# CloudEngineHub/MARL-LLM

Measured on AMD Instinct MI355X. Metric: agent-steps/sec, higher is better.
Workload: dtype f64 (state, every index / flag / reward decision) + f32 (obs, prior, action I/O, pre-filters); 1 GPU; assembly env, 64 agents x 4096 envs per GPU (64 x 4096 total), assembled state, prior-policy actions; agents=64, envs_per_gpu=4096, envs_total=4096, obs_dtype=f32, state_dtype=f64, seed=226, parallelism=env-sharded x1, no collective on the step path

## Files before the change

### marl_llm_amd/csrc/swarm_env.hip

```cpp

#include <hip/hip_runtime.h>

#include <cmath>
#include <cstdint>
#include <cstring>
#include <string>
#include <type_traits>
#include <utility>

#include "swarm_env.h"
#include "env_types.h"

using namespace swarm_internal;

namespace {

typedef unsigned long long u64;

typedef float f2v __attribute__((ext_vector_type(2)));

template <typename T> struct Pair;
template <> struct Pair<float>  { typedef float2 type; };
template <> struct Pair<double> { typedef double2 type; };
typedef __attribute__((ext_vector_type(2))) __bf16 bf2v;
// ... 60 lines not shown
        "v_addc_co_u32_e64 %2, %8, %2, %2, %8\n\t"
        "v_addc_co_u32_e64 %3, %9, %3, %3, %9\n\t"
        "v_addc_co_u32_e64 %4, %10, %4, %4, %10\n\t"
        "v_addc_co_u32_e64 %5, %11, %5, %5, %11"
        : "+v"(nb), "+v"(hi), "+v"(ht), "+v"(cd), "+v"(c1), "+v"(c2), "=&s"(m0), "=&s"(m1), "=&s"(m2), "=&s"(m3), "=&s"(m4), "=&s"(m5)
        : "v"(d2u), "v"(d2), "s"(c_nb), "s"(c_hi), "s"(c_ht), "s"(c_cd), "s"(c_c1), "s"(c_c2));
}

template <typename F, int... I>
__device__ __forceinline__ void static_for_impl(F &&f, std::integer_sequence<int, I...>)
{
    (f(std::integral_constant<int, I>{}), ...);
}
template <int N, typename F>
__device__ __forceinline__ void static_for(F &&f)
{
    static_for_impl(static_cast<F &&>(f), std::make_integer_sequence<int, N>{});
}

__device__ __forceinline__ double clamp_ref(double v, double lo, double hi)
{
    double m = (hi < v) ? hi : v;
    return (lo < m) ? m : lo;
}

#define REPS(k) ((P.dbg_phase == (k)) ? P.dbg_extra + 1 : 1)
#define FENCE() asm volatile("" ::: "memory")
#define EXIT_AT(k) do { if (P.dbg_phase == 15 && P.dbg_extra == (k)) return; } while (0)

#ifdef SWARM_STAMPS
#define STAMP(k) do { __builtin_amdgcn_sched_barrier(0); if (P.stamps != nullptr && (threadIdx.x & 63) == 0) P.stamps[((size_t)blockIdx.x * (blockDim.x >> 6) + (threadIdx.x >> 6)) * 24 + (k)] = clock64(); __builtin_amdgcn_sched_barrier(0); } while (0)
#else
#define STAMP(k) do { } while (0)
#endif

template <int NPAD, bool HALF = false> struct Geo {
    static_assert(!HALF || NPAD < 64, "the half-occupied geometry is for N < 64");
    static constexpr int NPAD_ = NPAD; static constexpr bool HALF_ = HALF;
    static constexpr bool CT_MAP = NPAD >= 64 || HALF;
    static constexpr int AG = NPAD < 64 ? 64 : NPAD;
    static constexpr int EPB = NPAD < 64 ? (64 / NPAD) / (HALF ? 2 : 1) : 1;
    static constexpr int ACTW = NPAD < 64 ? EPB * NPAD : 64;
    static constexpr int LPA = HALF ? 8 : 4;
    static constexpr int AGW = 64 / LPA;
    static constexpr int NW = AG / 64;
    static constexpr int WPE = 4;
    static constexpr int T = AG * WPE;
#ifndef SWARM_WPS
#define SWARM_WPS 7
#endif
#ifndef SWARM_WPS_SMALL
#define SWARM_WPS_SMALL 6
#endif
#ifndef SWARM_WPS_128
#define SWARM_WPS_128 6
#endif
    static constexpr int WPS_LAT = NPAD == 64 ? SWARM_WPS : (NPAD < 64 ? SWARM_WPS_SMALL : (NPAD == 128 ? SWARM_WPS_128 : 1));
    static constexpr int WPS_GEN = NPAD == 64 ? 6 : (NPAD < 64 ? 5 : 1);
};

template <int NPAD, bool HALF> struct LatMap {
    typedef Geo<NPAD, HALF> G_;
    static constexpr int AG = G_::AG, EPB = G_::EPB, NW = G_::NW, WPE = G_::WPE, T = G_::T;
    static constexpr int NRC = 16;
    static constexpr int al(int bytes) { return (bytes + 15) & ~15; }
    static constexpr int mx(int a, int b) { return a > b ? a : b; }
    static constexpr int sp_bytes = 4 * AG * 8;
    static constexpr int hdr_bytes = AG * 16;
    static constexpr int rew_scratch_bytes = NW * 1536;
    static constexpr int srow_bytes = mx((NRC - 1) * AG * 4, rew_scratch_bytes);
    static constexpr int pcr_bytes = AG * NRC;
    static constexpr int partc_bytes = WPE * AG * 2;
    static constexpr int partd_bytes = (WPE - 1) * AG * 8;
    static constexpr int lat_bytes = EPB * 64 * (8 + 2);
    static constexpr int cov_bytes = EPB * 64 * 8;
    static constexpr int flag_bytes = AG;
    static constexpr int snei_bytes = AG * kNeiStride * 2;
    static constexpr int sncf_bytes = AG * 4;
    static constexpr int snear_bytes = NW > 1 ? NW * AG * 8 : 0;
    static constexpr int orow_bytes = NRC * AG * 4;
    static constexpr int pm_bytes = (NW == 1 ? WPE * 4 : 5) * NW * AG * 8;
    static constexpr int sp = 0;
    static constexpr int hdr = sp + al(sp_bytes);
    static constexpr int srow = hdr + al(hdr_bytes);
    static constexpr int pcr = srow + al(srow_bytes);
    static constexpr int partc = pcr + al(pcr_bytes);
    static constexpr int partd = partc + al(partc_bytes);
    static constexpr int lat = partd + al(partd_bytes);
    static constexpr int cov = lat + al(lat_bytes);
    static constexpr int flag = cov + al(cov_bytes);
    static constexpr int snei = flag + al(flag_bytes);
// ... 91 lines not shown
    unsigned *cov = reinterpret_cast<unsigned *>(smem + LO(cov));
    int *sflag = reinterpret_cast<int *>(smem + LO(flag));
    unsigned char *pc = smem + P.off_pc;
    constexpr int NRC = LM::NRC;
    float4 *hdr = reinterpret_cast<float4 *>(smem + LO(hdr));
    unsigned *srow = reinterpret_cast<unsigned *>(smem + LO(srow));
    unsigned char *pcr = smem + LO(pcr);
    u64 *covrow = reinterpret_cast<u64 *>(smem + LO(cov));
    unsigned char *perm = smem + LO(perm);
    unsigned *orow = reinterpret_cast<unsigned *>(smem + P.off_orow);

    if constexpr (FILT) {
        bool any_zero = false;
        for (int k = 0; k < EPB; ++k) {
            const int ek = blockIdx.x * EPB + k;
            any_zero = any_zero || P.lat[ek < P.n_env ? ek : P.n_env - 1].nrows == 0;
        }
        if (any_zero == LAT) return;
    }
    const int tid = threadIdx.x, lane = tid & 63;
    STAMP(0);
    const int at = tid % AG;
    const int sx = __builtin_amdgcn_readfirstlane((tid / AG + (int)blockIdx.x) % WPE);
    const int aw = at >> 6;
    auto flag_get = [&]() -> bool { return LAT ? ((reinterpret_cast<const unsigned *>(sflag)[at >> 2] >> ((at & 3) * 8)) & 1u) != 0 : (sflag[at] & 1) != 0; };
    const bool thr_on = NPAD >= 64 || at < ACTW;
    const int el = (NPAD < 64 && thr_on) ? at / NPAD : 0;
    const int i = NPAD < 64 ? at % NPAD : at;
    const int e = blockIdx.x * EPB + el;
    const int n_a = P.n_a;
    const bool act = thr_on && (e < P.n_env) && (i < n_a);
    const int es = e < P.n_env ? e : P.n_env - 1;
    const int ng = P.n_g[es];
    int ngb = ng;
    if (EPB > 1) {
        for (int k = 0; k < EPB; ++k) {
            const int ek = blockIdx.x * EPB + k;
            const int v = P.n_g[ek < P.n_env ? ek : P.n_env - 1];
            ngb = v > ngb ? v : ngb;
        }
    }
    const int W = (ngb + 31) >> 5;
    constexpr int SB = WPE > 1 ? 1 : 0;
    int w0 = W;
    if (WPE > 1) { w0 = (W - 2 * (WPE - 1)) / WPE; w0 = w0 < 0 ? 0 : w0; }
    auto mine = [&](int w) -> bool {
        if (WPE == 1) return true;
        if (w < w0) return sx == SB;
        const int o = (w - w0) % (WPE - 1);
        return sx == (o < SB ? o : o + 1);
    };
    const double2 *gce = P.cells_xy + (size_t)es * P.ng_max;
    auto cell64 = [&](int c) -> double2 { double2 g = gce[c < ng ? c : 0]; if (!(c < ng)) { g.x = kSentinel; g.y = kSentinel; } return g; };
    const float *cq_e = cxq + (size_t)el * P.cxq_stride;

    const size_t sbase = (size_t)es * 2 * n_a;
    double px = __builtin_nan(""), py = __builtin_nan(""), vx = 0.0, vy = 0.0;
    double ax = 0.0, ay = 0.0;
    double sf0x = 0.0, sf0y = 0.0;
    OT2 pri_now; pri_now.x = to_out<OT>(0.0); pri_now.y = to_out<OT>(0.0);
    const bool copy_prior = DO_STEP && P.with_prior && a_prior != nullptr;
    if (sx == 0 && act) {
        if (DO_STEP) { const double2 sfl = P.sf_next[(size_t)e * n_a + i]; sf0x = sfl.x; sf0y = sfl.y; }
        px = P.p[sbase + i]; py = P.p[sbase + n_a + i];
        vx = P.dp[sbase + i]; vy = P.dp[sbase + n_a + i];
        if (DO_STEP) {
// ... 367 lines not shown
            const bool c0 = fmaf(e0, e0, dy2) < ri2, c1 = fmaf(e1, e1, dy2) < ri2;
            MT acc = range(ao0, ao1);
            MT bnd = (MT)((c0 ? (MT)0 : (MT)1 << (ao0 & (MB - 1))) | (c1 ? (MT)0 : (MT)1 << (ao1 & (MB - 1)))) & acc & rowm;
            acc &= ~bnd;
            while (__any(bnd != 0)) {
                if (bnd != 0) {
                    const int a = ffs0(bnd);
                    bnd &= bnd - 1;
                    const int c = rst + popc(rowm & (MT)(((MT)1 << a) - 1));
                    const double2 g = cell64(c);
                    const double ex = g.x - px, ey = g.y - py;
                    if (ex * ex + ey * ey < cut) acc |= (MT)1 << a;
                }
            }
            return rowm & acc;
        };
        for (int rep = 0, reps = REPS(3); rep < reps; ++rep) {
            FENCE();
            for (int t = wr; t < P.lat_nrs; t += WS)
                srow[t * AG + at] = (unsigned)(row_sel(b0s + t, L.R, P.c_sen) >> ca0);
            const int b0c = (int)ceilf(bpf - (L.Rc + 2.0f * lat_m));
            for (int t = wr; t < P.lat_nrc; t += WS) {
                const MT selc = row_sel(b0c + t, L.Rc, P.c_occ);
                const int bq = b0c + t < 0 ? 0 : (b0c + t > 63 ? 63 : b0c + t);
                if (selc != 0) {
                    if constexpr (MB == 32) atomicOr(reinterpret_cast<unsigned *>(&covrow[el * 64 + bq]), (unsigned)selc);
                    else atomicOr(reinterpret_cast<unsigned long long *>(&covrow[el * 64 + bq]), (unsigned long long)selc);
                }
            }
            best32 = INFINITY; second32 = INFINITY; bc = 0;
            const int ar0 = (int)floorf(apf) + 1;
            const int a_r = ar0 < 0 ? 0 : (ar0 > MB - 1 ? MB - 1 : ar0);
            const MT lowm = (MT)(((MT)1 << a_r) - 1);
            const int nr_hi = EPB == 1 ? nrows : 64;
            auto row_cands = [&](int b, float &d2d, float &d2u, int &c_dn) {
                const MT rowm = (EPB == 1 || b < nrows) ? rowmask(b) : (MT)0;
                const float dy = (float)b - bpf, dy2 = dy * dy;
                const MT up = rowm >> a_r, dn = rowm & lowm;
                const int a_up = a_r + ffs0(up);
                const int a_dn = MB - 1 - (MB == 32 ? __clz((int)dn) : __clzll((long long)dn));
                const float dxu = (float)a_up - apf, dxd = (float)a_dn - apf;
                d2u = (act && up != 0) ? fmaf(dxu, dxu, dy2) : INFINITY;
                d2d = (act && dn != 0) ? fmaf(dxd, dxd, dy2) : INFINITY;
                c_dn = rs[b] + popc(dn) - 1;
            };
            for (int b = wr; b < nr_hi; b += WS) {
                float d2d, d2u; int c_dn;
                row_cands(b, d2d, d2u, c_dn);
                second32 = __builtin_amdgcn_fmed3f(best32, second32, d2d);
                bool lt = d2d < best32;
                best32 = lt ? d2d : best32; bc = lt ? c_dn : bc;
                second32 = __builtin_amdgcn_fmed3f(best32, second32, d2u);
                lt = d2u < best32;
                best32 = lt ? d2u : best32; bc = lt ? c_dn + 1 : bc;
            }
            const float lat_dlt = 1.2e-7f * fmaxf(fabsf(apf), fabsf(bpf)) + 2e-6f;
            const float tol = 6.0f * sqrtf(second32) * lat_dlt + 1e-9f;
            const bool unc_min = act && (wave_exact || (second32 < INFINITY && (second32 - best32) <= tol));
            if (__any(unc_min)) {
                if (unc_min) {
                    const float thr = wave_exact ? INFINITY : best32 + tol;
                    double bestd = INFINITY; int bcd = bc;
                    for (int b = wr; b < nr_hi; b += WS) {
                        float d2d, d2u; int c_dn;
                        row_cands(b, d2d, d2u, c_dn);
                        const bool td = d2d <= thr, tu = d2u <= thr && d2u < INFINITY;
                        if ((td && d2d < INFINITY) || tu) {
                            const double2 g0 = cell64((td && d2d < INFINITY) ? c_dn : 0), g1 = cell64(tu ? c_dn + 1 : 0);
                            const double e0x = g0.x - px, e0y = g0.y - py, e1x = g1.x - px, e1y = g1.y - py;
                            const double q0 = e0x * e0x + e0y * e0y, q1 = e1x * e1x + e1y * e1y;
                            if (td && d2d < INFINITY && q0 < bestd) { bestd = q0; bcd = c_dn; }
                            if (tu && q1 < bestd) { bestd = q1; bcd = c_dn + 1; }
                        }
                    }
                    bc = bcd;
                }
            }
        }
        };
        if (sx != SB || WPE == 1) { if (P.lat_n32) walk(0u); else walk((u64)0); }
    } else
    for (int rep = 0, reps = REPS(3); rep < reps; ++rep) {
    FENCE();
    best32 = INFINITY; second32 = INFINITY; bc = 0;
    for (int w = 0; w < W; ++w) {
        if (!mine(w)) continue;
        unsigned word = 0, rword = 0;
        int mlo = 0, mhi = 0;
        int bl = 0; const float best_in = best32;
        unsigned orw = 0;
        const unsigned nlo = (unsigned)nearby1, nhi = (unsigned)(nearby1 >> 32);
        u64 unc = 0;
        const float4 *cq = reinterpret_cast<const float4 *>(cq_e + w * 64);
        static_for<16>([&](auto prc) {
            constexpr int pr = decltype(prc)::value;
            const float4 q = cq[pr];
            const f2v gx = {q.x, q.y}, gy = {q.z, q.w};
            const f2v rx = gx - pxx, ry = gy - pyy;
            const f2v d2v = __builtin_elementwise_fma(rx, rx, ry * ry);
            static_for<2>([&](auto hc) {
                constexpr int hh = decltype(hc)::value;
                constexpr int b = 2 * pr + hh;
                const float d2 = hh ? d2v.y : d2v.x;
                second32 = __builtin_amdgcn_fmed3f(best32, second32, d2);
                const bool lt = d2 < best32;
                best32 = lt ? d2 : best32;
                bl = lt ? b : bl;
                const u64 m_slo = __ballot(d2 < P.csen_lo), m_shi = __ballot(d2 < P.csen_hi);
                const u64 m_olo = __ballot(d2 < P.cocc_lo), m_ohi = __ballot(d2 < P.cocc_hi);
                rword = shl1_or_mask(rword, m_slo);
                if constexpr (NW == 1) {
                    const unsigned t = ((unsigned)m_olo & nlo) | ((unsigned)(m_olo >> 32) & nhi);
                    orw = shl1_or_mask(orw, __ballot(t != 0));
// ... 46 lines not shown
                }
            }
            if (unc_min) bc = bcd;
        }
    }
    part_c[sx * AG + at] = (pc_t)bc;
    double *part_d = reinterpret_cast<double *>(smem + LO(partd));
    if constexpr (LAT) {
        if (sx != SB || WPE == 1) {
            const double2 g = cell64(bc);
            const double ex = g.x - px, ey = g.y - py;
            part_d[(WPE > 1 && sx > SB ? sx - 1 : sx) * AG + at] = ex * ex + ey * ey;
        }
    }
    STAMP(16);
    EXIT_AT(4);
    __syncthreads();
    STAMP(17);
    double best = INFINITY; bc = 0;
    for (int rep = 0, reps = REPS(12); rep < reps; ++rep) {
    FENCE();
    best = INFINITY; bc = 0;
#pragma unroll
    for (int s = 0; s < WPE; ++s) {
        if (LAT && WPE > 1 && s == SB) continue;
        const int c = part_c[s * AG + at];
        double d;
        if constexpr (LAT) d = part_d[(WPE > 1 && s > SB ? s - 1 : s) * AG + at];
        else { const double2 g = cell64(c); const double ex = g.x - px, ey = g.y - py; d = ex * ex + ey * ey; }
        if (d < best || (d == best && c < bc)) { best = d; bc = c; }
    }
    }
    const bool in_shape = act && best < P.c_in[es];
    if (sx == 0) {
        sncf[at] = bc | (in_shape ? (1 << 30) : 0);
        if (P.export_small && act) {
            P.near_cell[(size_t)e * n_a + i] = bc;
            P.in_flag[(size_t)e * n_a + i] = in_shape ? 1 : 0;
        }
    }
    STAMP(4);
    EXIT_AT(5);

    const int PPR = P.obs_dim >> 1;
    const int HP = 2 * (P.with_self + P.topo) + 2;
    const int envs_here = (P.n_env - blockIdx.x * EPB) < EPB ? (P.n_env - blockIdx.x * EPB) : EPB;
    const int rows = envs_here * n_a;
    OT2 *out = reinterpret_cast<OT2 *>(obs) + (size_t)blockIdx.x * EPB * n_a * PPR;

    auto prior_policy = [&]() {
    if (sx == SB && P.with_prior) {
        double qx = 0.0, qy = 0.0;
        double lx = 0.0, ly = 0.0;
        {
            const int ncf = sncf[at];
            double tx = px - px, ty = py - py;
            if (!(ncf >> 30)) { const double2 g = cell64(ncf & 0xFFFF); tx = g.x - px; ty = g.y - py; }
            const double dt_ = sqrt(tx * tx + ty * ty);
            if (dt_ > 0) { qx += P.pk_att * tx / dt_; qy += P.pk_att * ty / dt_; }
            lx = qx; ly = qy;
            double avx = 0.0, avy = 0.0; int cnt = 0;
#pragma unroll
            for (int k = 0; k < kTopoMax; ++k) {
                const int j = snei[at * kNeiStride + k];
                const bool used = j >= 0;
                const int tj = el * NPAD + (used ? j : 0);
                const double x = px - sp[tj], y = py - sp[AG + tj];
                const double d2n = x * x + y * y;
                if (used && d2n > 0 && d2n < P.c_avoid) {
                    const double d = sqrt(d2n);
                    const double ux = x / d, uy = y / d;
                    const double factor = P.pk_rep * (P.r_avoid / d - 1.0);
// ... 947 lines not shown
```

### marl_llm_amd/csrc/env_api.hip

```cpp

#include <hip/hip_runtime.h>

#include <algorithm>
#include <cmath>
#include <cstddef>
#include <cstdint>
#include <cstring>
#include <new>
#include <string>
#include <utility>
#include <vector>

#include "swarm_env.h"
#include "env_types.h"

using namespace swarm_internal;

namespace {

thread_local std::string g_create_error;

double cut_lt(double t)
{
    if (!(t > 0)) return 0.0;
// ... 92 lines not shown
    h->path_mode = (!any_walk || h->lattice_disabled || k.lat_nrs > 15 || (any_scan && demote)) ? PATH_SCAN : any_scan ? PATH_MIXED : PATH_WALK;
    k.lattice = h->path_mode != PATH_SCAN ? 1 : 0;
    k.path_filter = 0;
    {
        const double dx = 1.2e-5, R = std::fmax(1.0, (double)rmax), thr = 0.05 * R / k.d_sen;
        const double dpsi_R = 2.4675 * 2.0 * std::sqrt(2.0) * dx + 1.2e-6 * R;
        k.rew_ga_lat = (float)(1.3 * (dpsi_R + dx + thr * dpsi_R / R));
        k.rew_gb_lat = (float)(4e-6 * R / k.d_sen);
    }
    {
        const int epb_full = h->npad < 64 ? 64 / h->npad : 1;
        const long long grid_full = ((long long)h->cfg.n_env + epb_full - 1) / epb_full;
        h->half = h->path_mode == PATH_WALK && h->npad < 64 && epb_full >= 2 && !(h->cfg.debug_flags & 4) && 2 * grid_full <= (long long)h->n_cu * 6;
    }
    env_layout(k, h->npad, h->half);
}

int export_pass(swarm_env *h, bool lists, bool cap_even)
{
    if (lists && !h->d_exp_occ) {
        const size_t EN = (size_t)h->cfg.n_env * h->cfg.n_agents;
        DevBuf<int> sensed, occ;
        HIP_ALLOC(h, sensed, EN * (size_t)h->kp.g_max);
        HIP_ALLOC(h, occ, EN * (size_t)h->kp.occ_max);
        h->d_exp_sensed = std::move(sensed); h->d_exp_occ = std::move(occ);
    }
    h->kp.export_small = 1; h->kp.cap_even = cap_even;
    if (lists) { h->kp.export_idx = 1; h->kp.exp_sensed = h->d_exp_sensed.get(); h->kp.exp_occ = h->d_exp_occ.get(); }
    const int rc = env_launch(h, false, nullptr, 0, nullptr, nullptr, nullptr, nullptr);
    h->kp.export_idx = 0; h->kp.export_small = 0; h->kp.cap_even = 0;
    return rc;
}

LatInfo classify_cells(const swarm_env *h, const double *gx, const double *gy, int n, LatEnv &L)
{
    std::memset(&L, 0, sizeof(L));
    if (h->lattice_disabled || !detect_lattice(gx, gy, n, L)) {
        std::memset(&L, 0, sizeof(L));
        return LatInfo{false, false, true, 0.0f, 0.0f, 0};
    }
    const double l = L.R;
    L.R = (float)(h->kp.d_sen / l); L.Rc = (float)((h->kp.r_avoid / 2.0) / l);
    const LatInfo info = {true, window_rows(L.R) <= 15, window_rows(L.R) > 15, L.R, L.Rc, L.ncols};
    if (!info.walk) std::memset(&L, 0, sizeof(L));
    return info;
}

LatInfo lattice_mode_of(swarm_env *h, const LatInfo *first, const LatInfo *last)
{
    LatInfo m = {true, false, false, 0.0f, 0.0f, 0};
    for (; first != last; ++first) {
        m.ok = m.ok && first->ok; m.scan = m.scan || first->scan;
        if (!first->walk) continue;
        m.walk = true;
        m.R = std::max(m.R, first->R); m.Rc = std::max(m.Rc, first->Rc);
        m.ncols = std::max(m.ncols, first->ncols);
    }
    set_lattice_mode(h, m.walk, m.scan, m.R, m.Rc, m.ncols);
    return m;
}

ShapeSet shape_set(const swarm_env *h)
{
    ShapeSet S;
    S.n_shapes = h->n_shapes; S.cells = h->d_shape_cells.get(); S.n_g = h->d_shape_ng.get(); S.l_cell = h->d_shape_l.get();
    S.c_in = h->d_shape_cin.get(); S.lat = h->d_shape_lat.get();
    return S;
}

int interleave(swarm_env *h, int e0, int count)
{
    HIP_LAUNCHED(h, launch_interleave(h->stream, h->d_cells.get(), h->d_cells_xy.get(), h->kp.ng_max, e0, count));
    return SWARM_OK;
}

}
// ... 139 lines not shown
            k.cap_shift = l - 1;
            const unsigned long long xmax = 2ull * (k.g_max - 1) * (unsigned long long)k.ng_max + k.g_max;
            k.cap_int = (((k.g_max - 1) & 1) == 1 && xmax < (1ull << 32) && l >= 1) ? 1 : 0;
        }
        k.dbg_phase = (cfg->debug_flags >> 8) & 0xF;
        k.dbg_extra = (cfg->debug_flags >> 12) & 0xF;
    }
    env_layout(k, h->npad, false);

    DeviceGuard g(dev);
    if (!g.ok) { delete h; return fail(nullptr, SWARM_ERR_HIP, "hipSetDevice failed"); }
    hipDeviceProp_t prop;
    if (hipGetDeviceProperties(&prop, dev) != hipSuccess) { delete h; return fail(nullptr, SWARM_ERR_HIP, "hipGetDeviceProperties failed"); }
    h->n_cu = prop.multiProcessorCount > 0 ? prop.multiProcessorCount : 256;
    if ((size_t)k.smem_generic > 160 * 1024) {
        delete h;
        return fail(nullptr, SWARM_ERR_INVALID, "configuration needs more LDS per workgroup than the device has (reduce n_cells_max / num_obs_grid_max)");
    }
    const size_t E = (size_t)cfg->n_env, N = (size_t)cfg->n_agents;
    hipError_t a = hipSuccess;
    auto alloc = [&](auto &buf, size_t count, int fill = -1) {
        if (a == hipSuccess) a = buf.alloc(count);
        if (a == hipSuccess && fill >= 0) a = hipMemset(buf.get(), fill, count * sizeof(*buf.get()));
    };
    alloc(h->d_p, E * 2 * N); alloc(h->d_dp, E * 2 * N);
    alloc(h->d_cells, E * 2 * (size_t)k.ng_max, 0); alloc(h->d_cin, E);
    alloc(h->d_cells_xy, E * (size_t)k.ng_max, 0);
    alloc(h->d_ng, E, 0); alloc(h->d_shape_idx, E, 0xFF);
    alloc(h->d_prior, E * N * 16, 0);
    if (cfg->llm_action) alloc(h->d_act_next, E * N, 0);
    alloc(h->d_lat, E);
    alloc(h->d_nei, E * N * (size_t)k.topo, 0xFF); alloc(h->d_near, E * N, 0);
    alloc(h->d_inflag, E * N, 0); alloc(h->d_sf, E * N, 0);
    if (a == hipSuccess) a = hipEventCreate(&h->ev0);
    if (a == hipSuccess) a = hipEventCreate(&h->ev1);
    if (a != hipSuccess) {
        std::string m = std::string("device allocation failed: ") + hipGetErrorString(a);
        swarm_destroy(h);
        return fail(nullptr, SWARM_ERR_HIP, m);
    }
    k.p = h->d_p.get(); k.dp = h->d_dp.get(); k.nei = h->d_nei.get(); k.near_cell = h->d_near.get(); k.in_flag = h->d_inflag.get(); k.sf_next = h->d_sf.get();
    k.prior_next = h->d_prior.get(); k.act_next = h->d_act_next.get();
    k.cells = h->d_cells.get(); k.cells_xy = h->d_cells_xy.get(); k.n_g = h->d_ng.get(); k.c_in = h->d_cin.get();
    k.lat = h->d_lat.get(); k.lattice = 0; k.lat_rw = k.lat_cw = 0; k.lat_nrs = k.lat_nrc = 0; k.lat_n32 = 0;
    k.c_near_hi = k.c_near * (1.0 + 1e-9);
    *out = h;
    return SWARM_OK;
}

int swarm_destroy(swarm_env_t *h)
{
    if (!h) return SWARM_OK;
    DeviceGuard g(h->device);
    (void)hipStreamSynchronize(h->stream);
    if (h->ev0) (void)hipEventDestroy(h->ev0);
    if (h->ev1) (void)hipEventDestroy(h->ev1);
    if (h->aux_stream) { (void)hipStreamSynchronize(h->aux_stream); (void)hipStreamDestroy(h->aux_stream); }
    if (h->ev_fork) (void)hipEventDestroy(h->ev_fork);
    if (h->ev_join) (void)hipEventDestroy(h->ev_join);
    delete h;
    return SWARM_OK;
}

int swarm_set_stream(swarm_env_t *h, void *s)
{
    if (!h) return SWARM_ERR_INVALID;
    h->stream = static_cast<hipStream_t>(s);
    return SWARM_OK;
}

int swarm_synchronize(swarm_env_t *h)
{
    if (!h) return SWARM_ERR_INVALID;
    DeviceGuard g(h->device);
    HIP_TRY(h, hipStreamSynchronize(h->stream));
    return SWARM_OK;
}

int swarm_obs_dim(const swarm_env_t *h) { return h ? h->kp.obs_dim : -1; }

int swarm_set_cells(swarm_env_t *h, int env_begin, int count, const double *cells, const int32_t *n_g, const double *l_cell)
{
    if (!h) return SWARM_ERR_INVALID;
    if (!cells || !n_g || !l_cell) return fail(h, SWARM_ERR_INVALID, "swarm_set_cells: null argument");
    if (env_begin < 0 || count < 1 || env_begin + count > h->cfg.n_env) return fail(h, SWARM_ERR_INVALID, "swarm_set_cells: env range out of bounds");
    std::vector<double> cin((size_t)count);
    for (int k = 0; k < count; ++k) {
        if (n_g[k] < 1 || n_g[k] > h->cfg.n_cells_max) return fail(h, SWARM_ERR_INVALID, "swarm_set_cells: n_g must be in [1, n_cells_max]");
        if (!(l_cell[k] > 0)) return fail(h, SWARM_ERR_INVALID, "swarm_set_cells: l_cell must be positive");
        cin[(size_t)k] = cut_lt(std::sqrt(2) * l_cell[k] / 2);
    }
    DeviceGuard g(h->device);
    const size_t row = (size_t)2 * h->kp.ng_max;
    HIP_TRY(h, hipMemcpyAsync(h->d_cells.get() + (size_t)env_begin * row, cells, (size_t)count * row * 8, hipMemcpyDefault, h->stream));
    if (int rc = interleave(h, env_begin, count)) return rc;
    HIP_TRY(h, hipMemcpyAsync(h->d_ng.get() + env_begin, n_g, (size_t)count * 4, hipMemcpyHostToDevice, h->stream));
    HIP_TRY(h, hipMemsetAsync(h->d_shape_idx.get() + env_begin, 0xFF, (size_t)count * 4, h->stream));
    HIP_TRY(h, hipMemcpyAsync(h->d_cin.get() + env_begin, cin.data(), (size_t)count * 8, hipMemcpyHostToDevice, h->stream));
    HIP_TRY(h, hipStreamSynchronize(h->stream));
    {
        std::vector<double> hc((size_t)count * row);
        HIP_TRY(h, hipMemcpy(hc.data(), h->d_cells.get() + (size_t)env_begin * row, (size_t)count * row * 8, hipMemcpyDeviceToHost));
        std::vector<LatEnv> lat((size_t)count);
        for (int k = 0; k < count; ++k) {
            const double *gx = hc.data() + (size_t)k * row, *gy = gx + h->kp.ng_max;
            h->env_lat[(size_t)(env_begin + k)] = classify_cells(h, gx, gy, n_g[k], lat[(size_t)k]);
        }
        HIP_TRY(h, hipMemcpy(h->d_lat.get() + env_begin, lat.data(), (size_t)count * sizeof(LatEnv), hipMemcpyHostToDevice));
        lattice_mode_of(h, h->env_lat.data(), h->env_lat.data() + h->env_lat.size());
    }
    for (int k = 0; k < count; ++k) h->cells_set[(size_t)(env_begin + k)] = 1;
    h->have_cells = true;
    for (char c : h->cells_set) if (!c) { h->have_cells = false; break; }
    h->observed = false;
    return SWARM_OK;
}

int swarm_set_shapes(swarm_env_t *h, int n_shapes, const double *shape_cells, const int32_t *n_g, const double *l_cell)
{
    if (!h) return SWARM_ERR_INVALID;
    if (n_shapes < 1 || !shape_cells || !n_g || !l_cell) return fail(h, SWARM_ERR_INVALID, "swarm_set_shapes: bad argument");
    const size_t row = (size_t)2 * h->kp.ng_max;
    std::vector<double> cin((size_t)n_shapes);
    std::vector<LatEnv> lat((size_t)n_shapes);
    std::vector<LatInfo> info((size_t)n_shapes);
    for (int k = 0; k < n_shapes; ++k) {
        if (n_g[k] < 1 || n_g[k] > h->cfg.n_cells_max) return fail(h, SWARM_ERR_INVALID, "swarm_set_shapes: n_g must be in [1, n_cells_max]");
        if (!(l_cell[k] > 0)) return fail(h, SWARM_ERR_INVALID, "swarm_set_shapes: l_cell must be positive");
        cin[(size_t)k] = cut_lt(std::sqrt(2) * l_cell[k] / 2);
        const double *gx = shape_cells + (size_t)k * row, *gy = gx + h->kp.ng_max;
        info[(size_t)k] = classify_cells(h, gx, gy, n_g[k], lat[(size_t)k]);
    }
    DeviceGuard g(h->device);
    const size_t S = (size_t)n_shapes;
    DevBuf<double> d_cells, d_l, d_cin; DevBuf<int> d_ng; DevBuf<LatEnv> d_lat;
    HIP_ALLOC(h, d_cells, S * row); HIP_ALLOC(h, d_l, S); HIP_ALLOC(h, d_cin, S); HIP_ALLOC(h, d_ng, S); HIP_ALLOC(h, d_lat, S);
    HIP_TRY(h, hipMemcpy(d_cells.get(), shape_cells, S * row * 8, hipMemcpyHostToDevice));
    HIP_TRY(h, hipMemcpy(d_l.get(), l_cell, S * 8, hipMemcpyHostToDevice));
    HIP_TRY(h, hipMemcpy(d_cin.get(), cin.data(), S * 8, hipMemcpyHostToDevice));
    HIP_TRY(h, hipMemcpy(d_ng.get(), n_g, S * 4, hipMemcpyHostToDevice));
    HIP_TRY(h, hipMemcpy(d_lat.get(), lat.data(), S * sizeof(LatEnv), hipMemcpyHostToDevice));
    h->d_shape_cells = std::move(d_cells); h->d_shape_l = std::move(d_l); h->d_shape_cin = std::move(d_cin);
    h->d_shape_ng = std::move(d_ng); h->d_shape_lat = std::move(d_lat);
    h->n_shapes = n_shapes; h->shape_lat = std::move(info);
    return SWARM_OK;
}

int swarm_reset(swarm_env_t *h, uint64_t seed, uint64_t episode, int64_t env_offset, void *obs)
{
    if (!h) return SWARM_ERR_INVALID;
    if (h->n_shapes < 1) return fail(h, SWARM_ERR_STATE, "swarm_reset: no shape set (swarm_set_shapes)");
    DeviceGuard g(h->device);
    HIP_LAUNCHED(h, launch_reset(h->stream, h->kp, shape_set(h), seed, episode, env_offset, h->d_cells.get(), h->d_ng.get(), h->d_cin.get(), h->d_lat.get(), h->d_shape_idx.get()));
    if (int rc = interleave(h, 0, h->cfg.n_env)) return rc;
    std::fill(h->cells_set.begin(), h->cells_set.end(), 1);
    h->have_cells = h->have_state = true;
    const LatInfo all = lattice_mode_of(h, h->shape_lat.data(), h->shape_lat.data() + h->shape_lat.size());
    std::fill(h->env_lat.begin(), h->env_lat.end(), all);
    h->observed = false;
    return swarm_observe(h, obs);
}

int swarm_select_shape(swarm_env_t *h, int32_t shape_index, void *obs)
{
// ... 284 lines not shown
```

### marl_llm_amd/csrc/env_types.h

```cpp
#ifndef SWARM_ENV_TYPES_H
#define SWARM_ENV_TYPES_H

#include <hip/hip_runtime.h>

#include <cstdint>
#include <string>
#include <vector>

#include "swarm_env.h"
#include "swarm_internal.h"

namespace swarm_internal __attribute__((visibility("hidden"))) {

constexpr int kTopoMax = 6;
constexpr int kNeiStride = 8;
constexpr double kSentinel = 1.0e200;

struct LatEnv {
    double ox, oy;
    double uxi, uyi, vxi, vyi;
    float R, Rc;
    int nrows, ncols;
    short rowstart[64];
    unsigned long long rowmask[64];
// ... 16 lines not shown
    float rew_ga, rew_gb;
    int force_exact;
    int cap_int;
    unsigned cap_magic; int cap_shift;
    int cap_even;
    int dbg_phase, dbg_extra;
    int off_cxyf, off_partc, off_lat, off_cov, off_flag;
    int off_hdr, off_srow, off_pcr, off_perm, off_rres, off_orow, off_partd;
    float rew_ga_lat, rew_gb_lat;
    float rew_thr_k;
    int lattice;
    int lat_rw, lat_cw;
    int lat_nrs, lat_nrc;
    int lat_n32;
    double c_near_hi;
    const LatEnv *lat;
    double d_sen, r_avoid, size_a, size2, k_ball, k_wall, c_wall, vel_max, dt;
    double bx0, by1, bx2, by3, w_half, h_half;
    double *p, *dp;
    int *nei, *near_cell, *in_flag;
    double2 *sf_next;
    const double *cells;
    const double2 *cells_xy;
    const int *n_g;
    const double *c_in;
    int *exp_sensed, *exp_occ;
    void *prior_next;
    double pk_att, pk_rep, pk_ali;
    double pk_llm;
    int llm;
    double2 *act_next;
    long long *stamps;
    int path_filter;
};

struct ShapeSet {
    int n_shapes;
    const double *cells;
    const int *n_g;
    const double *l_cell;
    const double *c_in;
    const LatEnv *lat;
};

struct LatInfo {
    bool ok, walk, scan;
    float R, Rc;
    int ncols;
};

enum PathMode { PATH_SCAN = 0, PATH_WALK = 1, PATH_MIXED = 2 };

}

struct swarm_env {
    template <class T, bool PINNED = false> using Buf = swarm_internal::DevBuf<T, PINNED>;
    swarm_config_t cfg = {};
    swarm_internal::KP kp = {};
    int device = 0, npad = 0;
    hipStream_t stream = nullptr;
    hipEvent_t ev0 = nullptr, ev1 = nullptr;
    bool have_cells = false, have_state = false, observed = false;
    int attr_smem[48];
    bool half = false;
    int path_mode = swarm_internal::PATH_SCAN;
    hipStream_t aux_stream = nullptr;
    hipEvent_t ev_fork = nullptr, ev_join = nullptr;
    int n_cu = 256;
    std::vector<char> cells_set;
    std::string err;
    Buf<double> d_p, d_dp, d_cells, d_cin;
    Buf<double2> d_cells_xy;
    Buf<swarm_internal::LatEnv> d_lat;
    int n_shapes = 0;
    Buf<double> d_shape_cells, d_shape_l, d_shape_cin;
    Buf<int> d_shape_ng, d_shape_idx;
    Buf<swarm_internal::LatEnv> d_shape_lat;
    std::vector<swarm_internal::LatInfo> shape_lat;
    std::vector<swarm_internal::LatInfo> env_lat;
    bool lattice_disabled = false;
    Buf<int> d_nei, d_near, d_inflag, d_ng;
    Buf<int> d_exp_sensed, d_exp_occ;
    Buf<double2> d_sf;
    Buf<char> d_prior;
    Buf<double2> d_act_next;
    Buf<double2> d_act64;
    Buf<char> d_io_obs, d_io_prior, d_io_action; Buf<float> d_io_rew; Buf<uint8_t> d_io_done; Buf<double> d_io_block;
    Buf<double, true> h_io_block[2]; Buf<char, true> h_io_action;
    size_t io_block_bytes = 0;
};

namespace swarm_internal __attribute__((visibility("hidden"))) {

int fail(swarm_env *h, int code, const std::string &msg);

#define HIP_TRY_AS(h, what, call)                                                             \
    do {                                                                                       \
        hipError_t e__ = (call);                                                               \
        if (e__ != hipSuccess)                                                                 \
            return swarm_internal::fail(h, SWARM_ERR_HIP, std::string(what) + ": " + hipGetErrorString(e__)); \
    } while (0)
#define HIP_TRY(h, call) HIP_TRY_AS(h, #call, call)
#define HIP_LAUNCHED(h, call) HIP_TRY_AS(h, "hipGetLastError()", call)
#define HIP_ALLOC(h, buf, count) HIP_TRY_AS(h, std::string((buf).kCall) + "(" #buf ")", (buf).alloc(count))

void env_layout(KP &k, int npad, bool half);
int env_launch(swarm_env *h, bool do_step, const void *action, int act_f64, void *obs, float *reward, uint8_t *done, void *a_prior);

hipError_t launch_reset(hipStream_t st, const KP &kp, const ShapeSet &S, unsigned long long seed, unsigned long long episode,
                        long long env_offset, double *cells, int *n_g, double *c_in, LatEnv *lat, int *shape_idx);
hipError_t launch_select_shape(hipStream_t st, const ShapeSet &S, int s, int ng_max, int n_env, double *cells, double2 *cells_xy,
                               int *n_g, double *c_in, LatEnv *lat, int *shape_idx);
hipError_t launch_interleave(hipStream_t st, const double *cells, double2 *cells_xy, int ng_max, int e0, int count);
hipError_t launch_metrics(hipStream_t st, const KP &kp, double *out);
hipError_t launch_metrics_step(hipStream_t st, const KP &kp, int n_cu, double *out);
hipError_t launch_export(hipStream_t st, int obs_dtype, const void *obs, const float *reward, const uint8_t *done,
// ... 6 lines not shown
```

Before: 3.140 billion agent-steps/s.

## Scan lattice rows outward from nearest row with early termination in nearest-cell search

Replaces the full scan over every lattice row in the nearest-cell search with an outward search that starts at the row nearest the agent and stops once the row distance exceeds the current best plus a tolerance. A full scan is kept for cases where the agent is far outside the grid or exact mode is set. The exact fp64 refinement pass uses the same bounded outward walk and adds a lowest-index tie-break. This cuts per-row work for agents near the lattice, at the cost of wave-wide __any checks per iteration and more divergent control flow.

New measurement: 3.168 billion agent-steps/s (median of 6 runs). No clear change (+0.9%).

```diff
diff --git a/marl_llm_amd/csrc/swarm_env.hip b/marl_llm_amd/csrc/swarm_env.hip
--- a/marl_llm_amd/csrc/swarm_env.hip
+++ b/marl_llm_amd/csrc/swarm_env.hip
@@ -731,45 +731,81 @@
             const int ar0 = (int)floorf(apf) + 1;
             const int a_r = ar0 < 0 ? 0 : (ar0 > MB - 1 ? MB - 1 : ar0);
             const MT lowm = (MT)(((MT)1 << a_r) - 1);
-            const int nr_hi = EPB == 1 ? nrows : 64;
-            auto row_cands = [&](int b, float &d2d, float &d2u, int &c_dn) {
-                const MT rowm = (EPB == 1 || b < nrows) ? rowmask(b) : (MT)0;
-                const float dy = (float)b - bpf, dy2 = dy * dy;
+            auto row_cands = [&](int b, bool on, float dy2, float &d2d, float &d2u, int &c_dn) {
+                const MT rowm = on ? rowmask(b) : (MT)0;
                 const MT up = rowm >> a_r, dn = rowm & lowm;
                 const int a_up = a_r + ffs0(up);
                 const int a_dn = MB - 1 - (MB == 32 ? __clz((int)dn) : __clzll((long long)dn));
                 const float dxu = (float)a_up - apf, dxd = (float)a_dn - apf;
-                d2u = (act && up != 0) ? fmaf(dxu, dxu, dy2) : INFINITY;
-                d2d = (act && dn != 0) ? fmaf(dxd, dxd, dy2) : INFINITY;
+                d2u = up != 0 ? fmaf(dxu, dxu, dy2) : INFINITY;
+                d2d = dn != 0 ? fmaf(dxd, dxd, dy2) : INFINITY;
                 c_dn = rs[b] + popc(dn) - 1;
             };
-            for (int b = wr; b < nr_hi; b += WS) {
-                float d2d, d2u; int c_dn;
-                row_cands(b, d2d, d2u, c_dn);
-                second32 = __builtin_amdgcn_fmed3f(best32, second32, d2d);
-                bool lt = d2d < best32;
-                best32 = lt ? d2d : best32; bc = lt ? c_dn : bc;
-                second32 = __builtin_amdgcn_fmed3f(best32, second32, d2u);
-                lt = d2u < best32;
-                best32 = lt ? d2u : best32; bc = lt ? c_dn + 1 : bc;
-            }
+            auto take = [&](float d2, int c) {
+                second32 = __builtin_amdgcn_fmed3f(best32, second32, d2);
+                const bool lt = d2 < best32;
+                best32 = lt ? d2 : best32; bc = lt ? c : bc;
+            };
             const float lat_dlt = 1.2e-7f * fmaxf(fabsf(apf), fabsf(bpf)) + 2e-6f;
+            const int r0 = (int)fminf(fmaxf(rintf(bpf), 0.0f), (float)(nrows - 1));
+            const int nr_hi = EPB == 1 ? nrows : 64;
+            const float oxb = fmaxf(fmaxf(-apf, apf - (float)(ncols - 1)), 0.0f), oyb = fmaxf(fmaxf(-bpf, bpf - (float)(nrows - 1)), 0.0f);
+            const float far_lb = fminf(sqrtf(fmaf(oxb, oxb, oyb * oyb)) - oyb - 1.0f, (float)(r0 > nrows - 1 - r0 ? r0 : nrows - 1 - r0));
+            const bool plain = wave_exact || __any(act && 3.0f * far_lb > (float)nr_hi);
+            if (plain) {
+                for (int b = wr; b < nr_hi; b += WS) {
+                    float d2d, d2u; int c_dn;
+                    const float dy = (float)b - bpf;
+                    row_cands(b, act && (EPB == 1 || b < nrows), dy * dy, d2d, d2u, c_dn);
+                    take(d2d, c_dn); take(d2u, c_dn + 1);
+                }
+            } else {
+                for (int t = wr; ; t += WS) {
+                    const int bu = r0 + t, bd = r0 - t;
+                    const float dyu = (float)bu - bpf, dyd = (float)bd - bpf;
+                    const float du2 = dyu * dyu, dd2 = dyd * dyd;
+                    const bool lu = act && bu < nrows && !(du2 - (6.0f * fabsf(dyu) * lat_dlt + 1e-9f) > best32);
+                    const bool ld = act && t > 0 && bd >= 0 && !(dd2 - (6.0f * fabsf(dyd) * lat_dlt + 1e-9f) > best32);
+                    if (!__any(lu || ld)) break;
+                    float d2d, d2u, e2d, e2u; int c_dn, c_en;
+                    row_cands(bu < nrows ? bu : nrows - 1, lu, du2, d2d, d2u, c_dn);
+                    row_cands(bd > 0 ? bd : 0, ld, dd2, e2d, e2u, c_en);
+                    take(d2d, c_dn); take(d2u, c_dn + 1); take(e2d, c_en); take(e2u, c_en + 1);
+                }
+            }
             const float tol = 6.0f * sqrtf(second32) * lat_dlt + 1e-9f;
             const bool unc_min = act && (wave_exact || (second32 < INFINITY && (second32 - best32) <= tol));
             if (__any(unc_min)) {
                 if (unc_min) {
                     const float thr = wave_exact ? INFINITY : best32 + tol;
                     double bestd = INFINITY; int bcd = bc;
-                    for (int b = wr; b < nr_hi; b += WS) {
+                    auto exact_row = [&](int b, bool on, float dy2) {
                         float d2d, d2u; int c_dn;
-                        row_cands(b, d2d, d2u, c_dn);
-                        const bool td = d2d <= thr, tu = d2u <= thr && d2u < INFINITY;
-                        if ((td && d2d < INFINITY) || tu) {
-                            const double2 g0 = cell64((td && d2d < INFINITY) ? c_dn : 0), g1 = cell64(tu ? c_dn + 1 : 0);
+                        row_cands(b, on, dy2, d2d, d2u, c_dn);
+                        const bool td = d2d <= thr && d2d < INFINITY, tu = d2u <= thr && d2u < INFINITY;
+                        if (td || tu) {
+                            const double2 g0 = cell64(td ? c_dn : 0), g1 = cell64(tu ? c_dn + 1 : 0);
                             const double e0x = g0.x - px, e0y = g0.y - py, e1x = g1.x - px, e1y = g1.y - py;
                             const double q0 = e0x * e0x + e0y * e0y, q1 = e1x * e1x + e1y * e1y;
-                            if (td && d2d < INFINITY && q0 < bestd) { bestd = q0; bcd = c_dn; }
-                            if (tu && q1 < bestd) { bestd = q1; bcd = c_dn + 1; }
+                            if (td && (q0 < bestd || (q0 == bestd && c_dn < bcd))) { bestd = q0; bcd = c_dn; }
+                            if (tu && (q1 < bestd || (q1 == bestd && c_dn + 1 < bcd))) { bestd = q1; bcd = c_dn + 1; }
+                        }
+                    };
+                    if (plain) {
+                        for (int b = wr; b < nr_hi; b += WS) {
+                            const float dy = (float)b - bpf;
+                            exact_row(b, EPB == 1 || b < nrows, dy * dy);
+                        }
+                    } else {
+                        for (int t = wr; ; t += WS) {
+                            const int bu = r0 + t, bd = r0 - t;
+                            const float dyu = (float)bu - bpf, dyd = (float)bd - bpf;
+                            const float du2 = dyu * dyu, dd2 = dyd * dyd;
+                            const bool lu = bu < nrows && du2 <= thr, ld = t > 0 && bd >= 0 && dd2 <= thr;
+                            if (!(lu || ld)) break;
+#pragma unroll 1
+                            for (int s = 0; s < 2; ++s)
+                                exact_row(s == 0 ? (bu < nrows ? bu : nrows - 1) : (bd > 0 ? bd : 0), s == 0 ? lu : ld, s == 0 ? du2 : dd2);
                         }
                     }
                     bc = bcd;
```

## Restrict nearest-cell search to sensing-window rows, with a far-agent fallback scan

Applied to the files above, without the earlier changes.

For lattice envs with 64 agents, the nearest-cell candidate search reuses the sensing-window row selections instead of scanning every lattice row. This is enabled only when the previous step's count of agents outside the sensing radius is at or below a switch threshold. Agents with no cell inside the window get their nearest cell from a separate wave-cooperative full-row scan that uses DPP min reductions. A per-env far-count byte buffer is added to carry that count between steps. The change lowers per-agent row work in the common case, at the cost of extra branching, added state and a more complex correctness path. The lattice-walk classification also now requires the in-shape cutoff to be smaller than the sensing cutoff.

Measured after the change: 3.148 billion agent-steps/s before, 3.193 billion agent-steps/s after (median of 6 runs). 1.4% higher.

```diff
diff --git a/marl_llm_amd/csrc/env_api.hip b/marl_llm_amd/csrc/env_api.hip
--- a/marl_llm_amd/csrc/env_api.hip
+++ b/marl_llm_amd/csrc/env_api.hip
@@ -148,7 +148,7 @@
     return rc;
 }
 
-LatInfo classify_cells(const swarm_env *h, const double *gx, const double *gy, int n, LatEnv &L)
+LatInfo classify_cells(const swarm_env *h, const double *gx, const double *gy, int n, double l_cell, LatEnv &L)
 {
     std::memset(&L, 0, sizeof(L));
     if (h->lattice_disabled || !detect_lattice(gx, gy, n, L)) {
@@ -157,7 +157,8 @@
     }
     const double l = L.R;
     L.R = (float)(h->kp.d_sen / l); L.Rc = (float)((h->kp.r_avoid / 2.0) / l);
-    const LatInfo info = {true, window_rows(L.R) <= 15, window_rows(L.R) > 15, L.R, L.Rc, L.ncols};
+    const bool walks = window_rows(L.R) <= 15 && cut_lt(std::sqrt(2) * l_cell / 2) < h->kp.c_sen;
+    const LatInfo info = {true, walks, !walks, L.R, L.Rc, L.ncols};
     if (!info.walk) std::memset(&L, 0, sizeof(L));
     return info;
 }
@@ -363,6 +364,7 @@
     alloc(h->d_lat, E);
     alloc(h->d_nei, E * N * (size_t)k.topo, 0xFF); alloc(h->d_near, E * N, 0);
     alloc(h->d_inflag, E * N, 0); alloc(h->d_sf, E * N, 0);
+    alloc(h->d_far, (E + 3) & ~(size_t)3, 0);
     if (a == hipSuccess) a = hipEventCreate(&h->ev0);
     if (a == hipSuccess) a = hipEventCreate(&h->ev1);
     if (a != hipSuccess) {
@@ -371,6 +373,7 @@
         return fail(nullptr, SWARM_ERR_HIP, m);
     }
     k.p = h->d_p.get(); k.dp = h->d_dp.get(); k.nei = h->d_nei.get(); k.near_cell = h->d_near.get(); k.in_flag = h->d_inflag.get(); k.sf_next = h->d_sf.get();
+    k.far_prev = h->d_far.get();
     k.prior_next = h->d_prior.get(); k.act_next = h->d_act_next.get();
     k.cells = h->d_cells.get(); k.cells_xy = h->d_cells_xy.get(); k.n_g = h->d_ng.get(); k.c_in = h->d_cin.get();
     k.lat = h->d_lat.get(); k.lattice = 0; k.lat_rw = k.lat_cw = 0; k.lat_nrs = k.lat_nrc = 0; k.lat_n32 = 0;
@@ -435,7 +438,7 @@
         std::vector<LatEnv> lat((size_t)count);
         for (int k = 0; k < count; ++k) {
             const double *gx = hc.data() + (size_t)k * row, *gy = gx + h->kp.ng_max;
-            h->env_lat[(size_t)(env_begin + k)] = classify_cells(h, gx, gy, n_g[k], lat[(size_t)k]);
+            h->env_lat[(size_t)(env_begin + k)] = classify_cells(h, gx, gy, n_g[k], l_cell[k], lat[(size_t)k]);
         }
         HIP_TRY(h, hipMemcpy(h->d_lat.get() + env_begin, lat.data(), (size_t)count * sizeof(LatEnv), hipMemcpyHostToDevice));
         lattice_mode_of(h, h->env_lat.data(), h->env_lat.data() + h->env_lat.size());
@@ -460,7 +463,7 @@
         if (!(l_cell[k] > 0)) return fail(h, SWARM_ERR_INVALID, "swarm_set_shapes: l_cell must be positive");
         cin[(size_t)k] = cut_lt(std::sqrt(2) * l_cell[k] / 2);
         const double *gx = shape_cells + (size_t)k * row, *gy = gx + h->kp.ng_max;
-        info[(size_t)k] = classify_cells(h, gx, gy, n_g[k], lat[(size_t)k]);
+        info[(size_t)k] = classify_cells(h, gx, gy, n_g[k], l_cell[k], lat[(size_t)k]);
     }
     DeviceGuard g(h->device);
     const size_t S = (size_t)n_shapes;
diff --git a/marl_llm_amd/csrc/env_types.h b/marl_llm_amd/csrc/env_types.h
--- a/marl_llm_amd/csrc/env_types.h
+++ b/marl_llm_amd/csrc/env_types.h
@@ -72,6 +72,7 @@
     double2 *act_next;
     long long *stamps;
     int path_filter;
+    unsigned char *far_prev;
 };
 
 struct ShapeSet {
@@ -122,6 +123,7 @@
     Buf<int> d_nei, d_near, d_inflag, d_ng;
     Buf<int> d_exp_sensed, d_exp_occ;
     Buf<double2> d_sf;
+    Buf<unsigned char> d_far;
     Buf<char> d_prior;
     Buf<double2> d_act_next;
     Buf<double2> d_act64;
diff --git a/marl_llm_amd/csrc/swarm_env.hip b/marl_llm_amd/csrc/swarm_env.hip
--- a/marl_llm_amd/csrc/swarm_env.hip
+++ b/marl_llm_amd/csrc/swarm_env.hip
@@ -116,6 +116,10 @@
 #define STAMP(k) do { __builtin_amdgcn_sched_barrier(0); if (P.stamps != nullptr && (threadIdx.x & 63) == 0) P.stamps[((size_t)blockIdx.x * (blockDim.x >> 6) + (threadIdx.x >> 6)) * 24 + (k)] = clock64(); __builtin_amdgcn_sched_barrier(0); } while (0)
 #else
 #define STAMP(k) do { } while (0)
+#endif
+
+#ifndef SWARM_FAR_SWITCH
+#define SWARM_FAR_SWITCH 8
 #endif
 
 template <int NPAD, bool HALF = false> struct Geo {
@@ -141,6 +145,11 @@
 #endif
     static constexpr int WPS_LAT = NPAD == 64 ? SWARM_WPS : (NPAD < 64 ? SWARM_WPS_SMALL : (NPAD == 128 ? SWARM_WPS_128 : 1));
     static constexpr int WPS_GEN = NPAD == 64 ? 6 : (NPAD < 64 ? 5 : 1);
+#ifdef SWARM_NC_ALLROWS
+    static constexpr bool NC_WIN = false;
+#else
+    static constexpr bool NC_WIN = NPAD == 64;
+#endif
 };
 
 template <int NPAD, bool HALF> struct LatMap {
@@ -298,6 +307,10 @@
     const bool act = thr_on && (e < P.n_env) && (i < n_a);
     const int es = e < P.n_env ? e : P.n_env - 1;
     const int ng = P.n_g[es];
+    constexpr bool NCW = LAT && G_::NC_WIN;
+    static_assert(!NCW || (EPB == 1 && NW == 1), "window-row candidates: one env per workgroup, one wave per split");
+    bool nc_win = false;
+    if constexpr (NCW) nc_win = ((reinterpret_cast<const unsigned *>(P.far_prev)[es >> 2] >> ((es & 3) * 8)) & 0xFFu) <= SWARM_FAR_SWITCH;
     int ngb = ng;
     if (EPB > 1) {
         for (int k = 0; k < EPB; ++k) {
@@ -777,7 +790,137 @@
             }
         }
         };
-        if (sx != SB || WPE == 1) { if (P.lat_n32) walk(0u); else walk((u64)0); }
+        auto walk_win = [&](auto tag, auto win_c) {
+        typedef decltype(tag) MT;
+        constexpr bool WIN = decltype(win_c)::value;
+        constexpr int MB = (int)sizeof(MT) * 8;
+        auto rowmask = [&](int b) -> MT { return MB == 32 ? (MT)reinterpret_cast<const unsigned *>(rm)[2 * b] : (MT)rm[b]; };
+        auto popc = [](MT v) -> int { return MB == 32 ? __popc((unsigned)v) : __popcll((unsigned long long)v); };
+        auto ffs0 = [](MT v) -> int { return (MB == 32 ? __ffs((unsigned)v) : __ffsll((unsigned long long)v)) - 1; };
+        auto range = [](int lo, int hi) -> MT { return hi >= lo ? (MT)((~(MT)0 >> (MB - 1 - hi)) & (~(MT)0 << lo)) : (MT)0; };
+        struct RowX { MT rowm; int rst; float dy2; };
+        auto row_sel = [&](int b, float rho, double cut, RowX &x) -> MT {
+            const bool rowok = act && b >= 0 && b < nrows;
+            const float dy = (float)b - bpf, dy2 = dy * dy;
+            const float ro = rho + lat_m, ri = rho - lat_m, ri2 = ri > 0.0f ? ri * ri : 0.0f;
+            const float ho2 = ro * ro - dy2;
+            const bool any_o = rowok && ho2 > 0.0f;
+            const float ho = __builtin_amdgcn_sqrtf(fmaxf(ho2, 0.0f));
+            int ao0 = (int)ceilf(apf - ho), ao1 = (int)floorf(apf + ho);
+            ao0 = ao0 < 0 ? 0 : ao0; ao1 = ao1 > ncols - 1 ? ncols - 1 : ao1;
+            const int bq = b < 0 ? 0 : (b > 63 ? 63 : b);
+            const MT rowm = any_o ? rowmask(bq) : (MT)0;
+            const int rst = rs[bq];
+            const float e0 = (float)ao0 - apf, e1 = (float)ao1 - apf;
+            const bool c0 = fmaf(e0, e0, dy2) < ri2, c1 = fmaf(e1, e1, dy2) < ri2;
+            MT acc = range(ao0, ao1);
+            MT bnd = (MT)((c0 ? (MT)0 : (MT)1 << (ao0 & (MB - 1))) | (c1 ? (MT)0 : (MT)1 << (ao1 & (MB - 1)))) & acc & rowm;
+            acc &= ~bnd;
+            x.rowm = rowm; x.rst = rst; x.dy2 = dy2;
+            while (__any(bnd != 0)) {
+                if (bnd != 0) {
+                    const int a = ffs0(bnd);
+                    bnd &= bnd - 1;
+                    const int c = rst + popc(rowm & (MT)(((MT)1 << a) - 1));
+                    const double2 g = cell64(c);
+                    const double ex = g.x - px, ey = g.y - py;
+                    if (ex * ex + ey * ey < cut) acc |= (MT)1 << a;
+                }
+            }
+            return rowm & acc;
+        };
+        for (int rep = 0, reps = REPS(3); rep < reps; ++rep) {
+            FENCE();
+            best32 = INFINITY; second32 = INFINITY; bc = 0;
+            const int ar0 = (int)floorf(apf) + 1;
+            const int a_r = ar0 < 0 ? 0 : (ar0 > MB - 1 ? MB - 1 : ar0);
+            const MT lowm = (MT)(((MT)1 << a_r) - 1);
+            auto cands_of = [&](MT cols, MT rowm, int rst, float dy2, float &d2d, float &d2u, int &c_dn) {
+                const MT up = cols >> a_r, dn = cols & lowm;
+                const int a_up = a_r + ffs0(up);
+                const int a_dn = MB - 1 - (MB == 32 ? __clz((int)dn) : __clzll((long long)dn));
+                const float dxu = (float)a_up - apf, dxd = (float)a_dn - apf;
+                d2u = (act && up != 0) ? fmaf(dxu, dxu, dy2) : INFINITY;
+                d2d = (act && dn != 0) ? fmaf(dxd, dxd, dy2) : INFINITY;
+                c_dn = rst + popc(rowm & lowm) - 1;
+            };
+            auto track = [&](float d2d, float d2u, int c_dn) {
+                second32 = __builtin_amdgcn_fmed3f(best32, second32, d2d);
+                bool lt = d2d < best32;
+                best32 = lt ? d2d : best32; bc = lt ? c_dn : bc;
+                second32 = __builtin_amdgcn_fmed3f(best32, second32, d2u);
+                lt = d2u < best32;
+                best32 = lt ? d2u : best32; bc = lt ? c_dn + 1 : bc;
+            };
+            for (int t = wr; t < P.lat_nrs; t += WS) {
+                RowX x;
+                const MT sel = row_sel(b0s + t, L.R, P.c_sen, x);
+                srow[t * AG + at] = (unsigned)(sel >> ca0);
+                if constexpr (WIN) {
+                    float d2d, d2u; int c_dn;
+                    cands_of(sel, x.rowm, x.rst, x.dy2, d2d, d2u, c_dn);
+                    track(d2d, d2u, c_dn);
+                }
+            }
+            const int b0c = (int)ceilf(bpf - (L.Rc + 2.0f * lat_m));
+            for (int t = wr; t < P.lat_nrc; t += WS) {
+                RowX x;
+                const MT selc = row_sel(b0c + t, L.Rc, P.c_occ, x);
+                const int bq = b0c + t < 0 ? 0 : (b0c + t > 63 ? 63 : b0c + t);
+                if (selc != 0) {
+                    if constexpr (MB == 32) atomicOr(reinterpret_cast<unsigned *>(&covrow[el * 64 + bq]), (unsigned)selc);
+                    else atomicOr(reinterpret_cast<unsigned long long *>(&covrow[el * 64 + bq]), (unsigned long long)selc);
+                }
+            }
+            const int nr_hi = WIN ? P.lat_nrs : (EPB == 1 ? nrows : 64);
+            auto row_cands = [&](int k, float &d2d, float &d2u, int &c_dn) {
+                if constexpr (WIN) {
+                    const int b = b0s + k, bq = b < 0 ? 0 : (b > 63 ? 63 : b);
+                    const MT sel = (MT)((MT)(srow[k * AG + at] & 0x1FFFFu) << (ca0 & (MB - 1)));
+                    const float dy = (float)b - bpf;
+                    cands_of(sel, rowmask(bq), rs[bq], dy * dy, d2d, d2u, c_dn);
+                } else {
+                    const MT rowm = (EPB == 1 || k < nrows) ? rowmask(k) : (MT)0;
+                    const float dy = (float)k - bpf;
+                    cands_of(rowm, rowm, rs[k], dy * dy, d2d, d2u, c_dn);
+                }
+            };
+            if constexpr (!WIN)
+            for (int b = wr; b < nr_hi; b += WS) {
+                float d2d, d2u; int c_dn;
+                row_cands(b, d2d, d2u, c_dn);
+                track(d2d, d2u, c_dn);
+            }
+            const float lat_dlt = 1.2e-7f * fmaxf(fabsf(apf), fabsf(bpf)) + 2e-6f;
+            const float tol = 6.0f * sqrtf(second32) * lat_dlt + 1e-9f;
+            const bool unc_min = act && (wave_exact || (second32 < INFINITY && (second32 - best32) <= tol));
+            if (__any(unc_min)) {
+                if (unc_min) {
+                    const float thr = wave_exact ? INFINITY : best32 + tol;
+                    double bestd = INFINITY; int bcd = bc;
+                    for (int b = wr; b < nr_hi; b += WS) {
+                        float d2d, d2u; int c_dn;
+                        row_cands(b, d2d, d2u, c_dn);
+                        const bool td = d2d <= thr, tu = d2u <= thr && d2u < INFINITY;
+                        if ((td && d2d < INFINITY) || tu) {
+                            const double2 g0 = cell64((td && d2d < INFINITY) ? c_dn : 0), g1 = cell64(tu ? c_dn + 1 : 0);
+                            const double e0x = g0.x - px, e0y = g0.y - py, e1x = g1.x - px, e1y = g1.y - py;
+                            const double q0 = e0x * e0x + e0y * e0y, q1 = e1x * e1x + e1y * e1y;
+                            if (td && d2d < INFINITY && q0 < bestd) { bestd = q0; bcd = c_dn; }
+                            if (tu && q1 < bestd) { bestd = q1; bcd = c_dn + 1; }
+                        }
+                    }
+                    bc = bcd;
+                }
+            }
+        }
+        };
+        if (sx != SB || WPE == 1) {
+            bool win = false;
+            if constexpr (NCW) win = nc_win;
+            if (win) { if constexpr (NCW) { if (P.lat_n32) walk_win(0u, std::true_type{}); else walk_win((u64)0, std::true_type{}); } }
+            else { if (P.lat_n32) walk(0u); else walk((u64)0); }
+        }
     } else
     for (int rep = 0, reps = REPS(3); rep < reps; ++rep) {
     FENCE();
@@ -890,12 +1033,104 @@
     }
     }
     const bool in_shape = act && best < P.c_in[es];
-    if (sx == 0) {
+    bool far = false;
+    if constexpr (NCW) { if (nc_win) far = act && !(best < P.c_sen); }
+    if (sx == 0 && !far) {
         sncf[at] = bc | (in_shape ? (1 << 30) : 0);
         if (P.export_small && act) {
             P.near_cell[(size_t)e * n_a + i] = bc;
             P.in_flag[(size_t)e * n_a + i] = in_shape ? 1 : 0;
         }
+    }
+    if constexpr (NCW) {
+        u64 farm = 0;
+        if (nc_win) farm = __ballot(far);
+        if (sx == 0 && e < P.n_env) {
+            if (!nc_win) farm = __ballot(act && !(best < P.c_sen));
+            const int nf = __popcll(farm);
+            P.far_prev[e] = (unsigned char)(nf > 255 ? 255 : nf);
+        }
+        const int nfar = __popcll(farm);
+        auto far_scan = [&](auto tag) {
+            typedef decltype(tag) MT;
+            constexpr int MB = (int)sizeof(MT) * 8;
+            auto popc = [](MT v) -> int { return MB == 32 ? __popc((unsigned)v) : __popcll((unsigned long long)v); };
+            auto bcastd = [](double v, int t) -> double {
+                const u64 b = __builtin_bit_cast(u64, v);
+                const unsigned lo = (unsigned)__builtin_amdgcn_readlane((int)(unsigned)b, t);
+                const unsigned hi = (unsigned)__builtin_amdgcn_readlane((int)(unsigned)(b >> 32), t);
+                return __builtin_bit_cast(double, ((u64)hi << 32) | lo);
+            };
+            auto wave_min = [](float v) -> float {
+                auto dpp_min = [](float x, auto ctrl) -> float {
+                    const int y = __builtin_amdgcn_update_dpp(0, __builtin_bit_cast(int, x), decltype(ctrl)::value, 0xF, 0xF, false);
+                    return fminf(x, __builtin_bit_cast(float, y));
+                };
+                v = dpp_min(v, std::integral_constant<int, 0xB1>{});
+                v = dpp_min(v, std::integral_constant<int, 0x4E>{});
+                v = dpp_min(v, std::integral_constant<int, 0x141>{});
+                v = dpp_min(v, std::integral_constant<int, 0x140>{});
+                const int b = __builtin_bit_cast(int, v);
+                const float r0 = __builtin_bit_cast(float, __builtin_amdgcn_readlane(b, 0)), r1 = __builtin_bit_cast(float, __builtin_amdgcn_readlane(b, 16));
+                const float r2 = __builtin_bit_cast(float, __builtin_amdgcn_readlane(b, 32)), r3 = __builtin_bit_cast(float, __builtin_amdgcn_readlane(b, 48));
+                return fminf(fminf(r0, r1), fminf(r2, r3));
+            };
+            const int nrows = P.lat[es].nrows;
+            const MT rowm = lane < nrows ? (MB == 32 ? (MT)reinterpret_cast<const unsigned *>(lrm)[2 * lane] : (MT)lrm[lane]) : (MT)0;
+            const int rst = lrs[lane];
+            const float rowf = (float)lane;
+            u64 fm = farm;
+            for (int k = 0; fm != 0; ++k) {
+                const int f = __ffsll((unsigned long long)fm) - 1;
+                fm &= fm - 1;
+                if ((k & (WPE - 1)) != sx) continue;
+                const float4 hf = hdr[f];
+                const float apf = hf.x + (float)__float_as_int(hf.w), bpf = hf.y + (float)__float_as_int(hf.z);
+                const int ar0 = (int)floorf(apf) + 1;
+                const int a_r = ar0 < 0 ? 0 : (ar0 > MB - 1 ? MB - 1 : ar0);
+                const MT lowm = (MT)(((MT)1 << a_r) - 1);
+                const MT up = rowm >> a_r, dn = rowm & lowm;
+                const int a_up = a_r + (MB == 32 ? __ffs((unsigned)up) : __ffsll((unsigned long long)up)) - 1;
+                const int a_dn = MB - 1 - (MB == 32 ? __clz((int)dn) : __clzll((long long)dn));
+                const float dy = rowf - bpf, dy2 = dy * dy;
+                const float dxu = (float)a_up - apf, dxd = (float)a_dn - apf;
+                const float d2u = up != 0 ? fmaf(dxu, dxu, dy2) : INFINITY;
+                const float d2d = dn != 0 ? fmaf(dxd, dxd, dy2) : INFINITY;
+                const int c_dn = rst + popc(dn) - 1;
+                const float m = wave_min(fminf(d2d, d2u));
+                const float lat_dlt = 1.2e-7f * fmaxf(fabsf(apf), fabsf(bpf)) + 2e-6f;
+                const float thr = wave_exact ? INFINITY : m + (6.0f * (1.001f * __builtin_amdgcn_sqrtf(m) + 0.1f) * lat_dlt + 1e-9f);
+                const bool td = d2d <= thr && d2d < INFINITY, tu = d2u <= thr && d2u < INFINITY;
+                const u64 bd = __ballot(td), bu = __ballot(tu);
+                int cell;
+                if (__popcll(bd) + __popcll(bu) == 1) {
+                    const int src = __ffsll((unsigned long long)(bd | bu)) - 1;
+                    cell = __builtin_amdgcn_readlane(c_dn, src) + (bd != 0 ? 0 : 1);
+                } else {
+                    const double fx = bcastd(px, f), fy = bcastd(py, f);
+                    double q = INFINITY; int qc = 0;
+                    if (td || tu) {
+                        const double2 g0 = cell64(td ? c_dn : 0), g1 = cell64(tu ? c_dn + 1 : 0);
+                        const double e0x = g0.x - fx, e0y = g0.y - fy, e1x = g1.x - fx, e1y = g1.y - fy;
+                        const double q0 = e0x * e0x + e0y * e0y, q1 = e1x * e1x + e1y * e1y;
+                        if (td) { q = q0; qc = c_dn; }
+                        if (tu && q1 < q) { q = q1; qc = c_dn + 1; }
+                    }
+                    double bq_ = INFINITY; cell = 0;
+                    u64 h = bd | bu;
+                    while (h != 0) {
+                        const int l = __ffsll((unsigned long long)h) - 1;
+                        h &= h - 1;
+                        const double ql = bcastd(q, l); const int cl = __builtin_amdgcn_readlane(qc, l);
+                        if (ql < bq_) { bq_ = ql; cell = cl; }
+                    }
+                }
+                sncf[f] = cell;
+                if (P.export_small && lane == 0) { P.near_cell[(size_t)e * n_a + f] = cell; P.in_flag[(size_t)e * n_a + f] = 0; }
+            }
+        };
+        EXIT_AT(8);
+        if (nc_win && nfar > sx) { if (P.lat_n32) far_scan(0u); else far_scan((u64)0); }
     }
     STAMP(4);
     EXIT_AT(5);
```
